# LeapLabTHU/LAUDNet

Measured on AMD Instinct MI355X. Metric: images/sec, LAUD-ResNet101 @224 bs256 (dynamic-inference hot path), higher is better.
Workload: dtype bf16x3 (fp32 tensors; each fp32 product = 3 bf16 MFMA products of hi/lo splits, fp32 accumulate)

## Files before the change

include/ldn_hip.h:

```cpp
#ifndef LDN_HIP_H
#define LDN_HIP_H

#include <stddef.h>
#include <stdint.h>

#ifdef __cplusplus
extern "C" {
#endif

#define LDN_OK 0
#define LDN_EINVAL (-1)
#define LDN_EHIP (-2)

const char* ldn_last_error(void);
int ldn_version(void);
int ldn_debug_violations(int* count, int* first_code, int reset);
int ldn_plan_timeouts(int* count, int reset);
const int* ldn_fault_flag(void);
int ldn_device_cus(int* cus);
#define LDN_MATH_DEFAULT (-1)
#define LDN_MATH_FP32 0
#define LDN_MATH_BF16X3 1
int ldn_default_math_mode(void);

// ... 77 lines not shown
                      double static_flops, int n_blocks, float* st_out, float* perc, float* flops, void* stream);

int ldn_conv_image(const float* a, int lda, int B, int Hi, int Wi, int ksize, int stride, int Ho, int Wo,
                   const float* w, int cin, int cout, const int32_t* k_idx, const int32_t* k_cnt, int kgran,
                   const int32_t* n_idx, const int32_t* n_cnt, const float* scale, const float* shift,
                   int shift_classes, const float* post_sub, int relu, const float* residual, int ldr,
                   float* out, int ldo, float* colsum, int out_format, int math_mode, void* stream);

int ldn_bottleneck_head(const float* x, int ldx, int B, int HW, int cin, const void* w1_split, int width,
                        const int32_t* ch_idx, const int32_t* ch_cnt, const float* scale1, const float* shift1,
                        const float* post_sub1, void* h1_split, int ldh, void* stream);
int ldn_bottleneck_head_f32(const float* x, int ldx, int B, int HW, int cin, const float* w1, int width,
                            const int32_t* ch_idx, const int32_t* ch_cnt, const float* scale1, const float* shift1,
                            const float* post_sub1, float* h1, int ldh, void* stream);
int ldn_bottleneck_tail_f32(const void* h1, int ldh, int B, int H, int Wd, int stride, int width, const void* w2_pairs_f32,
                            const void* w3_pairs_f32, int cout, const int32_t* ch_idx, const int32_t* ch_cnt, const float* scale2,
                            const float* shift2_tab, const float* post_sub2, const float* shift3, const float* residual,
                            int ldr, float* out, int ldo, float* colsum, void* stream);
int ldn_bottleneck_tail_splits(int H, int Wd, int width, int stride);
int ldn_bottleneck_tail(const void* h1_split, int ldh, int B, int H, int Wd, int stride, int width, const void* w2_pairs,
                        const void* w3_pairs, int cout, const int32_t* ch_idx, const int32_t* ch_cnt, const float* scale2,
                        const float* shift2_tab, const float* post_sub2, const float* shift3, const float* residual,
                        int ldr, float* out, int ldo, float* colsum, void* stream);
size_t ldn_x_split_bytes(size_t pixels, int cin);
int ldn_bottleneck_head_split(const float* x, int ldx, int B, int HW, int cin, const void* w1_split, int width,
                              const int32_t* ch_idx, const int32_t* ch_cnt, const float* scale1, const float* shift1,
                              const float* post_sub1, void* h1_split, int ldh, void* x_split, void* stream);
int ldn_bottleneck_tail_proj_fits(int H, int Wd, int width, int cin);
int ldn_bottleneck_tail_proj(const void* h1_split, int ldh, int B, int H, int Wd, int width, const void* w2_pairs,
                             const void* w3_pairs, int cout, const int32_t* ch_idx, const int32_t* ch_cnt, const float* scale2,
                             const float* shift2_tab, const float* post_sub2, const float* shift3d, const void* x_split,
                             int cin, const void* wd_pairs, float* out, int ldo, float* colsum, void* stream);

int ldn_bottleneck_smallmap_fits(int H, int Wd, int cin, int width, int cout);
int ldn_bottleneck_smallmap(const float* x, int ldx, int B, int H, int Wd, int cin, int width, const void* w1_split,
                            const void* w2_pairs, const void* w3_pairs, int cout, const int32_t* ch_idx, const int32_t* ch_cnt,
                            const float* scale1, const float* shift1, const float* post_sub1, const float* scale2,
                            const float* shift2_tab, const float* post_sub2, const float* shift3, const float* residual, int ldr,
                            float* out, int ldo, float* colsum, void* stream);

typedef struct ldn_chain_block {
    const void* w1_split; const float* scale1; const float* shift1; const float* post_sub1;
    const void* w2_pairs; const void* w3_pairs; const float* scale2; const float* shift2_tab; const float* post_sub2;
    const float* shift3;
    const float* mw1; const float* mb1; const float* mw2; const float* mb2;
} ldn_chain_block;
int ldn_bottleneck_chain_fits(int H, int Wd, int C, int width, int hidden, int G);
int ldn_bottleneck_chain(const float* x_in, float* x_work, int ldx, int B, int H, int Wd, int C, int width,
                         const ldn_chain_block* blocks, int nblocks, int hidden, int G, int gran, const float* gap_in,
                         int gap_splits, float* colsum, float* masks, int32_t* ch_idx, int32_t* ch_cnt, void* h1_split,
                         int ldh, void* stream);
int ldn_bottleneck_chain_f32(const float* x_in, float* x_work, int ldx, int B, int H, int Wd, int C, int width,
                         const ldn_chain_block* blocks, int nblocks, int hidden, int G, int gran, const float* gap_in,
                         int gap_splits, float* colsum, float* masks, int32_t* ch_idx, int32_t* ch_cnt, float* h1,
                         int ldh, void* stream);

size_t ldn_stem_weight_bytes(int cout);
int ldn_stem_conv_pool(const float* x, int B, int H, int W, const void* w_frag, const float* shift, int cout, float* out,
                       int Hp, int Wp, void* stream);
int ldn_stem_gap_splits(int H, int W);
int ldn_stem_conv_pool_gap(const float* x, int B, int H, int W, const void* w_frag, const float* shift, int cout,
                           float* out, int Hp, int Wp, float* gap, void* stream);

size_t ldn_stem3_weight_bytes(int cout);
int ldn_stem3_conv(const float* x, int B, int H, int W, const void* w_frag, const float* shift, int cout, int relu, float* out,
                   int Ho, int Wo, void* stream);
// ... 49 lines not shown
```

laudnet_amd/_lib.py:

```python
from __future__ import annotations

import ctypes as C
import os

import torch

_PKG = os.path.dirname(os.path.abspath(__file__))
LIB_PATH = os.environ.get("LDN_LIB_PATH", os.path.join(_PKG, "libldn_hip.so"))

_P = C.c_void_p
_I = C.c_int

SIGNATURES = {
    "ldn_last_error": ([], C.c_char_p),
    "ldn_version": ([], _I),
    "ldn_debug_violations": ([C.POINTER(_I), C.POINTER(_I), _I], _I),
    "ldn_plan_timeouts": ([C.POINTER(_I), _I], _I),
    "ldn_fault_flag": ([], C.POINTER(_I)),
    "ldn_device_cus": ([C.POINTER(_I)], _I),
    "ldn_default_math_mode": ([], _I),
    "ldn_spatial_masker": ([_P, _I, _I, _I, _I, _P, _P, _I, _I, _P, _P, _P, _P, _P, _P], _I),
    "ldn_spatial_masker_workspace_bytes": ([_I, _I, _I, _I, _I], C.c_size_t),
    "ldn_mask_to_index": ([_P, _I, _I, _I, _I, _I, _I, _P, _P, _P, _P, _P, _P, _P, _P, _P, _P, _P], _I),
    "ldn_mask_to_index_workspace_bytes": ([_I, _I, _I, _I], C.c_size_t),
# ... 27 lines not shown
    "ldn_grouped16_weight_bytes": ([_I], C.c_size_t),
    "ldn_grouped16_conv3x3_rows": ([_P, _I, _P, _P, _I, _P, _I, _P, _P, _I, _P, _I, _P], _I),
    "ldn_grouped16_images_fit": ([_I, _I, _I], _I),
    "ldn_grouped16_conv3x3_images": ([_P, _I, _P, _I, _I, _I, _I, _I, _I, _P, _I, _P, _P, _I, _P, _I, _P], _I),
    "ldn_plan_work_zeroed": ([_I], _I),
    "ldn_coarsen_cell_means": ([_P, _I, _I, _I, _P, _P], _I),
    "ldn_grouped16_images_bands": ([_I, _I, _I, _I, _I], _I),
    "ldn_grouped16_conv3x3_images_gap": ([_P, _I, _P, _I, _I, _I, _I, _I, _I, _P, _I, _P, _P, _I, _P, _I, _P, _P], _I),
    "ldn_se_gate_slots": ([_P, _I, _P, _I, _I, _I, _I, _P, _P, _P, _P, _P, _P], _I),
    "ldn_conv_rows_gated": ([_P, _I, _P, _I, _P, _I, _I, _P, _P, _I, _P, _P, _P, _I, _P, _I, _P, _I, _P], _I),
    "ldn_grouped_conv3x3_image": ([_P, _I, _I, _I, _I, _I, _I, _I, _P, _I, _I, _P, _P, _P, _P, _I, _P, _I, _P], _I),
    "ldn_se_packed": ([_P, _I, _P, _I, _I, _I, _P, _P, _P, _P, _P, _P, _I, _P, _P], _I),
    "ldn_se_packed_workspace_bytes": ([_I, _I, _I], C.c_size_t),
    "ldn_conv_image": ([_P, _I, _I, _I, _I, _I, _I, _I, _I, _P, _I, _I, _P, _P, _I, _P, _P, _P, _P, _I, _P, _I,
                        _P, _I, _P, _I, _P, _I, _I, _P], _I),
    "ldn_bottleneck_head": ([_P, _I, _I, _I, _I, _P, _I, _P, _P, _P, _P, _P, _P, _I, _P], _I),
    "ldn_bottleneck_head_f32": ([_P, _I, _I, _I, _I, _P, _I, _P, _P, _P, _P, _P, _P, _I, _P], _I),
    "ldn_bottleneck_tail_splits": ([_I, _I, _I, _I], _I),
    "ldn_bottleneck_tail": ([_P, _I, _I, _I, _I, _I, _I, _P, _P, _I, _P, _P, _P, _P, _P, _P, _P, _I, _P, _I, _P, _P], _I),
    "ldn_bottleneck_tail_f32": ([_P, _I, _I, _I, _I, _I, _I, _P, _P, _I, _P, _P, _P, _P, _P, _P, _P, _I, _P, _I, _P, _P], _I),
    "ldn_x_split_bytes": ([C.c_size_t, _I], C.c_size_t),
    "ldn_bottleneck_head_split": ([_P, _I, _I, _I, _I, _P, _I, _P, _P, _P, _P, _P, _P, _I, _P, _P], _I),
    "ldn_bottleneck_tail_proj_fits": ([_I, _I, _I, _I], _I),
    "ldn_bottleneck_tail_proj": ([_P, _I, _I, _I, _I, _I, _P, _P, _I, _P, _P, _P, _P, _P, _P, _P, _I, _P, _P, _I, _P, _P], _I),
    "ldn_stem_weight_bytes": ([_I], C.c_size_t),
    "ldn_stem_conv_pool": ([_P, _I, _I, _I, _P, _P, _I, _P, _I, _I, _P], _I),
    "ldn_stem_gap_splits": ([_I, _I], _I),
    "ldn_stem_conv_pool_gap": ([_P, _I, _I, _I, _P, _P, _I, _P, _I, _I, _P, _P], _I),
    "ldn_stem3_weight_bytes": ([_I], C.c_size_t),
    "ldn_stem3_conv": ([_P, _I, _I, _I, _P, _P, _I, _I, _P, _I, _I, _P], _I),
    "ldn_packed_mha": ([_P, _I, _P, _P, _I, _I, _I, _I, C.c_float, _P, _I, _P], _I),
    "ldn_packed_mha_heads": ([_P, _I, _P, _P, _I, _I, _I, _I, C.c_float, _P, _P, _I, _P], _I),
    "ldn_bottleneck_chain_fits": ([_I, _I, _I, _I, _I, _I], _I),
    "ldn_bottleneck_smallmap_fits": ([_I, _I, _I, _I, _I], _I),
    "ldn_bottleneck_smallmap": ([_P, _I, _I, _I, _I, _I, _I, _P, _P, _P, _I, _P, _P, _P, _P, _P, _P, _P, _P, _P, _P, _I, _P, _I, _P, _P], _I),
    "ldn_bottleneck_chain": ([_P, _P, _I, _I, _I, _I, _I, _I, _P, _I, _I, _I, _I, _P, _I, _P, _P, _P, _P, _P, _I, _P], _I),
    "ldn_bottleneck_chain_f32": ([_P, _P, _I, _I, _I, _I, _I, _I, _P, _I, _I, _I, _I, _P, _I, _P, _P, _P, _P, _P, _I, _P], _I),
}

_lib = None


class LdnError(RuntimeError):
    pass


def load():
    global _lib
    if _lib is not None:
        return _lib
    if not os.path.exists(LIB_PATH):
        raise LdnError(f"{LIB_PATH} not found: build it with `python -m laudnet_amd.build` "
                       "(laudnet_amd has no CPU or PyTorch fallback for the hot path)")
    lib = C.CDLL(LIB_PATH)
    for name, (argtypes, restype) in SIGNATURES.items():
        fn = getattr(lib, name)
        fn.argtypes = argtypes
        fn.restype = restype
    _lib = lib
    return lib


def ptr(t):
    if t is None:
        return None
    return C.c_void_p(t.data_ptr())
# ... 55 lines not shown
```

laudnet_amd/csrc/ldn_small.hip:

```cpp
#include <type_traits>

#include "ldn_common.h"

namespace ldn {

typedef __bf16 bf16x8 __attribute__((ext_vector_type(8)));
typedef __bf16 bf16x2 __attribute__((ext_vector_type(2)));
typedef unsigned u32x2 __attribute__((ext_vector_type(2)));
typedef unsigned u32x4 __attribute__((ext_vector_type(4)));

struct SmallArgs {
    const float* x; int ldx;
    int B, H, Wd, HW, cin, W, cout;
    const unsigned char* w1s;
    const unsigned char* w2p;
    const unsigned char* w3p;
    const int32_t* k_idx; const int32_t* k_cnt;
    const float* sc1; const float* sh1; const float* ps1;
    const float* sc2; const float* sh2; const float* ps2;
    const float* sh3;
    const float* residual; int ldr; float* out; int ldo;
    float* colsum;
};

__device__ __attribute__((aligned(16))) float g_small_zero[4] = {0.f, 0.f, 0.f, 0.f};

#ifndef SM_ABLATE
#define SM_ABLATE 0
#endif
#ifdef LDN_TRACE
__device__ unsigned long long* g_small_trace = nullptr;
#define ST(x) x = __builtin_amdgcn_s_memtime();
// ... 93 lines not shown
    const int slot32 = 16 * g.w2row;
    if (SM_FORCE_K16 == 0 && 3 * slot32 <= g.space) { g.nks2 = 2; g.slot2 = slot32; g.d2 = g.space / slot32 < 3 ? g.space / slot32 : 3; }
    else { g.nks2 = 1; g.slot2 = 8 * g.w2row; g.d2 = g.space / g.slot2 < 4 ? g.space / g.slot2 : 4; }
    g.d3 = g.space / 32768 < 3 ? g.space / 32768 : 3;
    return g;
}

__device__ __forceinline__ void store_presplit(unsigned char* act, int HW, int j, int pm, int h, int qd, const f32x4 v) {
    const bf16x2 h0 = {(__bf16)v[0], (__bf16)v[1]}, h1 = {(__bf16)v[2], (__bf16)v[3]};
    const bf16x2 l0 = {(__bf16)(v[0] - (float)h0[0]), (__bf16)(v[1] - (float)h0[1])};
    const bf16x2 l1 = {(__bf16)(v[2] - (float)h1[0]), (__bf16)(v[3] - (float)h1[1])};
    const u32x2 hi = {__builtin_bit_cast(unsigned, h0), __builtin_bit_cast(unsigned, h1)};
    const u32x2 lo = {__builtin_bit_cast(unsigned, l0), __builtin_bit_cast(unsigned, l1)};
    const unsigned sw = ((unsigned)pm >> 1) & 7u;
    unsigned char* row = act + (size_t)j * HW * 128 + pm * 128;
    *reinterpret_cast<u32x2*>(row + (((2u * qd) ^ sw) << 4) + 8 * h) = hi;
    *reinterpret_cast<u32x2*>(row + (((2u * qd + 1u) ^ sw) << 4) + 8 * h) = lo;
}

__device__ __forceinline__ float half_sum_dpp(float v) {
    auto dpp = [](float x, auto ctrl, auto rmask) {
        return __builtin_bit_cast(float, __builtin_amdgcn_update_dpp(0, __builtin_bit_cast(int, x), decltype(ctrl)::value, decltype(rmask)::value, 0xf, false));
    };
    v += dpp(v, std::integral_constant<int, 0xB1>{}, std::integral_constant<int, 0xf>{});
    v += dpp(v, std::integral_constant<int, 0x4E>{}, std::integral_constant<int, 0xf>{});
    v += dpp(v, std::integral_constant<int, 0x141>{}, std::integral_constant<int, 0xf>{});
    v += dpp(v, std::integral_constant<int, 0x140>{}, std::integral_constant<int, 0xf>{});
    v += dpp(v, std::integral_constant<int, 0x142>{}, std::integral_constant<int, 0xa>{});
    return v;
}

}

__global__ __launch_bounds__(512, 2) void k_smallmap(const SmallArgs p) {
    extern __shared__ __attribute__((aligned(16))) unsigned char smem[];
    const int tid = threadIdx.x, lane = tid & 63;
    const int wave = __builtin_amdgcn_readfirstlane(tid >> 6);
    const int l31 = lane & 31, h = lane >> 5;
    const int t = wave & 1, q = wave >> 1;
    const int b = blockIdx.x;
    const int W = p.W, HW = p.HW;
#ifdef LDN_TRACE
    unsigned long long ts[6] = {0, 0, 0, 0, 0, 0}, ta = 0, tb = 0, wt[3] = {0, 0, 0}, ct[3] = {0, 0, 0}, x3[3] = {0, 0, 0};
    ST(ts[0])
#endif
    int* const s_kidx = reinterpret_cast<int*>(smem);
    unsigned char* const s_act = smem + S_ACT_OFF;

    const int Kb = min(p.k_cnt[b], W);
    const int nsub = __builtin_amdgcn_readfirstlane(ceil_div(Kb, 32));
    const int Kp = nsub * 32;
    for (int i = tid; i < W + 32; i += 512) s_kidx[i] = i < Kb ? p.k_idx[(size_t)b * W + i] : -1;
    if (tid < 32) reinterpret_cast<float*>(smem + S_ZERO_OFF)[tid] = 0.f;
    LDN_DCHECK(p.k_cnt[b] >= 0 && p.k_cnt[b] <= W && (p.k_cnt[b] & 1) == 0, 701);
    if (tid < Kb) {
        const int ch = p.k_idx[(size_t)b * W + tid];
        LDN_DCHECK(ch >= 0 && ch < W, 702);
        LDN_DCHECK((tid & 1) ? (ch == p.k_idx[(size_t)b * W + tid - 1] + 1) : ((ch & 1) == 0), 703);
        LDN_DCHECK(tid == 0 || ch > p.k_idx[(size_t)b * W + tid - 1], 704);
    }
    __syncthreads();

    SmallGeom G = small_geom(HW, nsub);
    G.d2 = __builtin_amdgcn_readfirstlane(G.d2); G.d3 = __builtin_amdgcn_readfirstlane(G.d3);
    G.nks2 = __builtin_amdgcn_readfirstlane(G.nks2); G.slot2 = __builtin_amdgcn_readfirstlane(G.slot2);
    G.w2row = __builtin_amdgcn_readfirstlane(G.w2row); G.ring_off = __builtin_amdgcn_readfirstlane(G.ring_off);
    const int pm = 32 * t + l31;
// ... 152 lines not shown
                    }
                }
            }
#pragma unroll
            for (int i = 0; i < 4; ++i)
#pragma unroll
                for (int r = 0; r < 16; ++r) acc[i][r] = 0.f;
            lds_barrier();
            ST(ts[2])
        }

        {
            const int oy = pm / p.Wd, ox = pm - oy * p.Wd;
            unsigned tmask = 0;
#pragma unroll
            for (int tp = 0; tp < 9; ++tp) {
                const int iy = oy + tp / 3 - 1, ix = ox + tp % 3 - 1;
                const bool ok = pvalid && iy >= 0 && iy < p.H && ix >= 0 && ix < p.Wd;
                tmask |= ok ? (1u << tp) : 0u;
            }
            const int cls = (((oy - 1 < 0) | ((oy + 1 >= p.H) << 1)) * 4 + ((ox - 1 < 0) | ((ox + 1 >= p.Wd) << 1)));
            const int nks = G.nks2, D = G.d2, W2ROW = G.w2row, slotB = G.slot2;
            const int nf = W2ROW / 1024;
            const int per = nks == 2 ? 1 : 2;
            const int nchunks = nsub * 9 * per;
            const int ipc = nks * nf;
            int npo[4];
#pragma unroll
            for (int f = 0; f < 4; ++f) {
                const int v = 64 * f + lane;
                const int ch = 2 * v < Kb ? s_kidx[2 * v] : -1;
                npo[f] = ch >= 0 ? (ch >> 1) * 16 : -1;
            }
            if (D > 1) {
                unsigned vo[4];
#pragma unroll
                for (int f = 0; f < 4; ++f) {
                    const int v = 64 * f + lane;
                    vo[f] = (unsigned)((s_kidx[2 * v < Kb ? 2 * v : 0] >> 1) * 16 + (3 - f) * 1024);
                }
                const long tapstride = (long)(W / 2) * (W / 2) * 16;
                const unsigned ring_bytes = (unsigned)(D * slotB);
                int is = 0, itp = 0, ihf = 0; unsigned foff = 0;
                int rbv[2];
                auto load_rb = [&]() {
#pragma unroll
                    for (int e = 0; e < 2; ++e)
                        rbv[e] = (s_kidx[min(32 * min(is, nsub - 1) + (nks == 2 ? 4 * wave + 2 * e : 16 * e + 2 * wave), Kb - 2)] >> 1) * (W / 2) * 16;
                };
                load_rb();
                auto row_dma = [&](const void* sbase, unsigned lds) {
                    if (nf == 3) dma16_gather_row<3>(vo, sbase, lds);
                    else if (nf == 4) dma16_gather_row<4>(vo, sbase, lds);
                    else if (nf == 2) dma16_gather_row<2>(vo, sbase, lds);
                    else dma16_gather_row<1>(vo, sbase, lds);
                };
                auto issue = [&]() {
                    const unsigned char* tapbase = p.w2p + (long)itp * tapstride - 3072;
                    const unsigned slot = lds_ring + foff;
                    if (nks == 2) {
                        row_dma(uniform_ptr(tapbase + __builtin_amdgcn_readfirstlane(rbv[0])), slot + (2 * wave) * W2ROW);
                        row_dma(uniform_ptr(tapbase + __builtin_amdgcn_readfirstlane(rbv[1])), slot + (2 * wave + 1) * W2ROW);
                    } else {
                        row_dma(uniform_ptr(tapbase + __builtin_amdgcn_readfirstlane(ihf ? rbv[1] : rbv[0])), slot + wave * W2ROW);
                    }
                    foff += slotB; if (foff == ring_bytes) foff = 0;
                    if (++ihf == per) { ihf = 0; if (++itp == 9) { itp = 0; ++is; load_rb(); } }
// ... 179 lines not shown
#pragma unroll
                                for (int qq = 0; qq < 4; ++qq) e[i][qq] = *reinterpret_cast<const u32x2*>(ws + a_lane + qq * W2ROW + jo[i]);
#pragma unroll
                            for (int i = 0; i < 4; ++i) {
                                if (q + 4 * i < nsub) {
                                    const u32x4 ahu = {e[i][0][0], e[i][1][0], e[i][2][0], e[i][3][0]};
                                    const u32x4 alu = {e[i][0][1], e[i][1][1], e[i][2][1], e[i][3][1]};
                                    const bf16x8 ah = __builtin_bit_cast(bf16x8, ahu), al = __builtin_bit_cast(bf16x8, alu);
                                    acc[i] = __builtin_amdgcn_mfma_f32_32x32x16_bf16(al, bh, acc[i], 0, 0, 0);
                                    acc[i] = __builtin_amdgcn_mfma_f32_32x32x16_bf16(ah, bl, acc[i], 0, 0, 0);
                                    acc[i] = __builtin_amdgcn_mfma_f32_32x32x16_bf16(ah, bh, acc[i], 0, 0, 0);
                                }
                                if (D > 1) issue_part(i);
                            }
                            if (D > 1) issue_advance();
                        }
                        ST(tb)
                        ST_ADD(ct[1], ta, tb)
                    }
                }
            }
            }
            wait_vm_n<0>();
            lds_barrier();
            ST(ts[3])
            float* const s_tab = reinterpret_cast<float*>(smem + G.ring_off);
            for (int i = tid; i < 18 * Kp; i += 512) {
                const int k = i / Kp, n = i - k * Kp;
                const int ch = s_kidx[n];
                const float* src = k == 0 ? p.sc2 : (k == 1 ? p.ps2 : p.sh2 + (size_t)(k - 2) * W);
                s_tab[i] = ch >= 0 ? src[ch] : 0.f;
            }
            lds_barrier();
            if (pvalid) {
#pragma unroll
                for (int i = 0; i < 4; ++i) {
                    const int j = q + 4 * i;
                    if (j < nsub) {
#pragma unroll
                        for (int qd = 0; qd < 4; ++qd) {
                            const int n0 = 32 * j + 8 * qd + 4 * h;
                            const f32x4 sc = *reinterpret_cast<const f32x4*>(s_tab + n0);
                            const f32x4 ps = *reinterpret_cast<const f32x4*>(s_tab + Kp + n0);
                            const f32x4 sh = *reinterpret_cast<const f32x4*>(s_tab + (2 + cls) * Kp + n0);
                            f32x4 v;
#pragma unroll
                            for (int e = 0; e < 4; ++e) v[e] = fmaxf(acc[i][4 * qd + e] * sc[e] + sh[e], 0.f) - ps[e];
                            store_presplit(s_act, HW, j, pm, h, qd, v);
                        }
                    }
                }
            }
            lds_barrier();
            ST(ts[4])
        }
    }

    {
        const int D = G.d3;
        const int nk16 = Kp / 16;
        const int ngroups = ceil_div(p.cout, 512);
        const int nchunks = ngroups * nk16;
        int ig = 0, iks = 0, ioff = 0, coff = 0;
        const unsigned char* i3base = nullptr;
        auto issue_begin = [&]() {
            i3base = nullptr;
            if (ig < ngroups && nk16 > 0) {
                const int kch = s_kidx[16 * iks + 2 * wave];
                if (kch >= 0) i3base = p.w3p + ((long)(kch >> 1) * p.cout + 512 * ig + 2 * lane) * 8;
            }
        };
        auto issue_part = [&](int f) {
            const unsigned slot = lds_ring + ioff;
            const unsigned char* src = (i3base && 512 * ig + 128 * f < p.cout) ? i3base + f * 1024 : reinterpret_cast<const unsigned char*>(g_small_zero);
            dma16(src, slot + wave * 4096 + f * 1024);
        };
        auto issue_advance = [&]() {
            ioff += 32768; if (ioff == D * 32768) ioff = 0;
            if (ig < ngroups && nk16 > 0) { if (++iks == nk16) { iks = 0; ++ig; } }
        };
        auto issue = [&]() {
            issue_begin();
#pragma unroll
            for (int f = 0; f < 4; ++f) issue_part(f);
            issue_advance();
        };
        const bool fast3 = D > 1 && (p.cout & 511) == 0 && nk16 > 0;
        if (D > 1 && !fast3) for (int c = 0; c < D - 1; ++c) issue();
        const unsigned rx = ((unsigned)prow >> 1) & 7u;
        const unsigned a_lane = (unsigned)(4 * h * 4096 + l31 * 8);
        auto group_epilogue = [&](int g) {
// ... 151 lines not shown
                        const u32x4 ahu = {e[i][0][0], e[i][1][0], e[i][2][0], e[i][3][0]};
                        const u32x4 alu = {e[i][0][1], e[i][1][1], e[i][2][1], e[i][3][1]};
                        const bf16x8 ah = __builtin_bit_cast(bf16x8, ahu), al = __builtin_bit_cast(bf16x8, alu);
                        acc[i] = __builtin_amdgcn_mfma_f32_32x32x16_bf16(al, bh, acc[i], 0, 0, 0);
                        acc[i] = __builtin_amdgcn_mfma_f32_32x32x16_bf16(ah, bl, acc[i], 0, 0, 0);
                        acc[i] = __builtin_amdgcn_mfma_f32_32x32x16_bf16(ah, bh, acc[i], 0, 0, 0);
                    }
                    if (D > 1) issue_part(i);
                }
                if (D > 1) issue_advance();
            }
            if (active) group_epilogue(g);
        }
        }
        wait_vm_n<0>();
#ifdef LDN_TRACE
        ST(ts[5])
        if (g_small_trace && lane == 0) {
            unsigned long long* r = g_small_trace + ((size_t)b * 8 + wave) * 16;
            for (int i = 0; i < 6; ++i) r[i] = ts[i];
            for (int i = 0; i < 3; ++i) { r[6 + i] = wt[i]; r[9 + i] = ct[i]; }
            r[12] = nsub; r[13] = x3[0]; r[14] = x3[1]; r[15] = x3[2];
        }
#endif
        if (p.colsum && !active) {
            for (int cch = 128 * q + lane * 2; cch < p.cout; cch += 512) {
                p.colsum[((size_t)b * 2 + t) * p.cout + cch] = 0.f;
                p.colsum[((size_t)b * 2 + t) * p.cout + cch + 1] = 0.f;
            }
        }
    }
}

LDN_DEFINE_TU_VIOLATIONS(tu_violations_small)

static bool small_fits(int HW, int cin, int width, int cout) {
    if (HW < 1 || HW > 64 || width < 64 || width > 512 || width % 64 || cin < 32 || cin % 32 || cout < 128 || cout % 128) return false;
    const int nsub = width / 32;
    const SmallGeom g = small_geom(HW, nsub);
    if (S_ACT_OFF + g.act_bytes > S_LDS - S_TAB1_BYTES) return false;
    if (g.space < 18 * width * 4) return false;
    if (g.d2 < 1 || g.d3 < 1) return false;
    if (2 * (64 + width) * 128 > S_LDS - S_ACT_OFF) return false;
    return true;
}

}

using namespace ldn;

#ifdef LDN_TRACE
extern "C" int ldn_debug_set_small_trace(void* buf) {
    unsigned long long* q = static_cast<unsigned long long*>(buf);
    return hipMemcpyToSymbol(HIP_SYMBOL(g_small_trace), &q, sizeof(q)) == hipSuccess ? 0 : -2;
}
#endif

extern "C" int ldn_bottleneck_smallmap_fits(int H, int Wd, int cin, int width, int cout) {
    if (H < 1 || Wd < 1) return 0;
    return small_fits(H * Wd, cin, width, cout) ? 1 : 0;
}

extern "C" int ldn_bottleneck_smallmap(const float* x, int ldx, int B, int H, int Wd, int cin, int width, const void* w1_split,
                                       const void* w2_pairs, const void* w3_pairs, int cout, const int32_t* ch_idx,
                                       const int32_t* ch_cnt, const float* scale1, const float* shift1, const float* post_sub1,
                                       const float* scale2, const float* shift2_tab, const float* post_sub2, const float* shift3,
                                       const float* residual, int ldr, float* out, int ldo, float* colsum, void* stream) {
    LDN_REQUIRE(x && w1_split && w2_pairs && w3_pairs && ch_idx && ch_cnt && scale1 && shift1 && post_sub1 && scale2 && shift2_tab &&
                post_sub2 && shift3 && out, "ldn_bottleneck_smallmap: null pointer");
    LDN_REQUIRE(B > 0 && H > 0 && Wd > 0, "ldn_bottleneck_smallmap: bad geometry");
    LDN_REQUIRE(small_fits(H * Wd, cin, width, cout),
                "ldn_bottleneck_smallmap: a %dx%d map with cin %d, width %d, cout %d does not fit the workgroup (ldn_bottleneck_smallmap_fits == 0)",
                H, Wd, cin, width, cout);
    LDN_REQUIRE(ldx >= cin && ldx % 4 == 0 && ldo >= cout && ldo % 4 == 0 && (!residual || (ldr >= cout && ldr % 4 == 0)),
                "ldn_bottleneck_smallmap: bad ldx / ldo / ldr");
    LDN_REQUIRE((uintptr_t)x % 16 == 0 && (uintptr_t)w1_split % 16 == 0 && (uintptr_t)w2_pairs % 16 == 0 && (uintptr_t)w3_pairs % 16 == 0 &&
                (uintptr_t)out % 16 == 0 && (uintptr_t)residual % 16 == 0 && (uintptr_t)shift3 % 16 == 0 && (uintptr_t)colsum % 16 == 0,
                "ldn_bottleneck_smallmap: pointers must be 16-byte aligned");
    SmallArgs a{};
    a.x = x; a.ldx = ldx; a.B = B; a.H = H; a.Wd = Wd; a.HW = H * Wd; a.cin = cin; a.W = width; a.cout = cout;
    a.w1s = static_cast<const unsigned char*>(w1_split);
    a.w2p = static_cast<const unsigned char*>(w2_pairs);
    a.w3p = static_cast<const unsigned char*>(w3_pairs);
    a.k_idx = ch_idx; a.k_cnt = ch_cnt;
    a.sc1 = scale1; a.sh1 = shift1; a.ps1 = post_sub1; a.sc2 = scale2; a.sh2 = shift2_tab; a.ps2 = post_sub2; a.sh3 = shift3;
    a.residual = residual; a.ldr = ldr; a.out = out; a.ldo = ldo; a.colsum = colsum;
    LDN_REQUIRE(allow_dynamic_lds(reinterpret_cast<const void*>(&k_smallmap), S_LDS), "k_smallmap: cannot reserve %d B of LDS", S_LDS);
    hipLaunchKernelGGL(k_smallmap, dim3((unsigned)B), dim3(512), S_LDS, static_cast<hipStream_t>(stream), a);
    LDN_CHECK_LAUNCH("k_smallmap");
    return LDN_OK;
}
```

laudnet_amd/ops.py:

```python
from __future__ import annotations

import os
import threading
import weakref
from dataclasses import dataclass

import torch

from . import _lib as L


def _f32c(t, what):
    if t is None:
        return None
    if t.dtype != torch.float32 or not t.is_contiguous():
        raise L.LdnError(f"{what}: expected a contiguous float32 tensor, got {t.dtype} strides {t.stride()}")
    return t


def _f32rows(t, what):
    if t is None:
        return None
    if t.dtype != torch.float32 or t.dim() != 2 or t.stride(1) != 1 or t.data_ptr() % 16 != 0:
        raise L.LdnError(f"{what}: expected a 16-byte aligned float32 matrix with contiguous rows, got {t.dtype} strides {t.stride()}")
# ... 871 lines not shown
    v = (t[:, :, :, 0] + t[:, :, :, 1]).permute(0, 3, 1, 2, 4).reshape(-1, cin)
    return v[:pixels]


def bottleneck_tail_proj_fits(H, W, width, cin):
    return bool(L.load().ldn_bottleneck_tail_proj_fits(H, W, width, cin))


def bottleneck_tail_proj(h1_split, w2_pairs, w3_pairs, ch_idx, ch_cnt, scale2, shift2_tab, post_sub2, shift3d, x_split, wd_pairs,
                         out_nhwc, *, colsum=None):
    L.require_device(h1_split, w2_pairs, w3_pairs, x_split, wd_pairs, out_nhwc)
    lib = L.load()
    B, H, Wd, ldh = h1_split.shape
    width = ch_idx.shape[1]
    cout = out_nhwc.shape[-1]
    cin = wd_pairs.shape[0] * 2
    if tuple(out_nhwc.shape) != (B, H, Wd, cout) or x_split.numel() * 4 < lib.ldn_x_split_bytes(B * H * Wd, cin) or not x_split.is_contiguous():
        raise L.LdnError(f"bottleneck_tail_proj: out must be [B={B}, {H}, {Wd}, cout], x_split the buffer bottleneck_head filled")
    for t in (w2_pairs, w3_pairs, wd_pairs):
        if t.dtype != torch.bfloat16 or not t.is_contiguous():
            raise L.LdnError("bottleneck_tail_proj: w2_pairs / w3_pairs / wd_pairs must be the contiguous bf16 tensors of pack_w2_pairs / pack_w3_pairs")
    L.check(lib.ldn_bottleneck_tail_proj(L.ptr(_f32c(h1_split, "h1")), ldh, B, H, Wd, width, L.ptr(w2_pairs), L.ptr(w3_pairs), cout,
                                         L.ptr(_i32c(ch_idx, "ch_idx")), L.ptr(_i32c(ch_cnt, "ch_cnt")), L.ptr(_f32c(scale2, "scale2")),
                                         L.ptr(_f32c(shift2_tab, "shift2_tab")), L.ptr(_f32c(post_sub2, "post_sub2")),
                                         L.ptr(_f32c(shift3d, "shift3d")), L.ptr(x_split), cin, L.ptr(wd_pairs),
                                         L.ptr(_f32c(out_nhwc, "out")), cout, L.ptr(colsum), L.stream_ptr(out_nhwc)), "ldn_bottleneck_tail_proj")
    return out_nhwc


def bottleneck_smallmap_fits(H, W, cin, width, cout):
    return bool(L.load().ldn_bottleneck_smallmap_fits(H, W, cin, width, cout))


def bottleneck_smallmap(x_nhwc, w1_split, w2_pairs, w3_pairs, ch_idx, ch_cnt, scale1, shift1, post_sub1, scale2, shift2_tab, post_sub2,
                        shift3, out_nhwc, *, residual=None, colsum=None):
    L.require_device(x_nhwc, w1_split, w2_pairs, w3_pairs, out_nhwc)
    lib = L.load()
    B, H, Wd, cin = x_nhwc.shape
    width = ch_idx.shape[1]
    cout = out_nhwc.shape[-1]
    if tuple(out_nhwc.shape) != (B, H, Wd, cout) or (residual is not None and tuple(residual.shape) != (B, H, Wd, cout)):
        raise L.LdnError(f"bottleneck_smallmap: out / residual must be [B={B}, {H}, {Wd}, cout]")
    if colsum is not None and (tuple(colsum.shape) != (B, 2, cout) or not colsum.is_contiguous()):
        raise L.LdnError("bottleneck_smallmap: colsum must be a contiguous [B, 2, cout] tensor")
    for w in (w1_split, w2_pairs, w3_pairs):
        if w.dtype != torch.bfloat16 or not w.is_contiguous():
            raise L.LdnError("bottleneck_smallmap: weights must be the contiguous bf16 tensors of pack_w1_split / pack_w2_pairs / pack_w3_pairs")
    L.check(lib.ldn_bottleneck_smallmap(L.ptr(_f32c(x_nhwc, "x")), cin, B, H, Wd, cin, width, L.ptr(w1_split), L.ptr(w2_pairs),
                                        L.ptr(w3_pairs), cout, L.ptr(_i32c(ch_idx, "ch_idx")), L.ptr(_i32c(ch_cnt, "ch_cnt")),
                                        L.ptr(_f32c(scale1, "scale1")), L.ptr(_f32c(shift1, "shift1")), L.ptr(_f32c(post_sub1, "post_sub1")),
                                        L.ptr(_f32c(scale2, "scale2")), L.ptr(_f32c(shift2_tab, "shift2_tab")),
                                        L.ptr(_f32c(post_sub2, "post_sub2")), L.ptr(_f32c(shift3, "shift3")), L.ptr(residual),
                                        cout if residual is not None else 0, L.ptr(_f32c(out_nhwc, "out")), cout, L.ptr(colsum),
                                        L.stream_ptr(out_nhwc)), "ldn_bottleneck_smallmap")
    return out_nhwc


def pack_stem_weights(w_scaled):
    cout = w_scaled.shape[0]
    if tuple(w_scaled.shape[1:]) != (3, 7, 7) or cout % 32:
        raise L.LdnError("pack_stem_weights: expected [cout % 32 == 0, 3, 7, 7]")
    w = w_scaled.detach().float().permute(0, 2, 3, 1).reshape(cout, 7, 21)
    k = torch.zeros(cout, 8, 24, device=w.device, dtype=torch.float32)
    k[:, :7, :21] = w
    k = k.reshape(cout, 24, 8)[:, :22]
    k = k.reshape(cout // 32, 32, 11, 2, 8)
# ... 79 lines not shown
```

Before: 23590.

## Add register-pipelined weight streaming variant of smallmap bottleneck kernel

Adds a templated variant of the small-feature-map bottleneck kernel. In it, the 3x3 conv and the final 1x1 conv stream weight fragments directly from global memory into a 4-deep register ring. These loads are software-pipelined against double-buffered LDS activation fragments feeding bf16x3 MFMAs, with each wave owning 64-pixel by 32/64-channel tiles. The goal is to hide global weight-load latency and avoid the previous staging path. It is selected by default through an environment variable. The trade-off is higher register pressure at 512 threads with 2 blocks per CU, which could cause spills.

```diff
diff --git a/include/ldn_hip.h b/include/ldn_hip.h
--- a/include/ldn_hip.h
+++ b/include/ldn_hip.h
@@ -133,6 +133,7 @@
                              const float* shift2_tab, const float* post_sub2, const float* shift3d, const void* x_split,
                              int cin, const void* wd_pairs, float* out, int ldo, float* colsum, void* stream);
 
+int ldn_bottleneck_smallmap_form(void);
 int ldn_bottleneck_smallmap_fits(int H, int Wd, int cin, int width, int cout);
 int ldn_bottleneck_smallmap(const float* x, int ldx, int B, int H, int Wd, int cin, int width, const void* w1_split,
                             const void* w2_pairs, const void* w3_pairs, int cout, const int32_t* ch_idx, const int32_t* ch_cnt,
diff --git a/laudnet_amd/_lib.py b/laudnet_amd/_lib.py
--- a/laudnet_amd/_lib.py
+++ b/laudnet_amd/_lib.py
@@ -83,6 +83,7 @@
     "ldn_packed_mha": ([_P, _I, _P, _P, _I, _I, _I, _I, C.c_float, _P, _I, _P], _I),
     "ldn_packed_mha_heads": ([_P, _I, _P, _P, _I, _I, _I, _I, C.c_float, _P, _P, _I, _P], _I),
     "ldn_bottleneck_chain_fits": ([_I, _I, _I, _I, _I, _I], _I),
+    "ldn_bottleneck_smallmap_form": ([], _I),
     "ldn_bottleneck_smallmap_fits": ([_I, _I, _I, _I, _I], _I),
     "ldn_bottleneck_smallmap": ([_P, _I, _I, _I, _I, _I, _I, _P, _P, _P, _I, _P, _P, _P, _P, _P, _P, _P, _P, _P, _P, _I, _P, _I, _P, _P], _I),
     "ldn_bottleneck_chain": ([_P, _P, _I, _I, _I, _I, _I, _I, _P, _I, _I, _I, _I, _P, _I, _P, _P, _P, _P, _P, _I, _P], _I),
diff --git a/laudnet_amd/csrc/ldn_small.hip b/laudnet_amd/csrc/ldn_small.hip
--- a/laudnet_amd/csrc/ldn_small.hip
+++ b/laudnet_amd/csrc/ldn_small.hip
@@ -1,3 +1,4 @@
+#include <stdlib.h>
 #include <type_traits>
 
 #include "ldn_common.h"
@@ -157,7 +158,7 @@
 
 }
 
-__global__ __launch_bounds__(512, 2) void k_smallmap(const SmallArgs p) {
+template <int REGW> __device__ __forceinline__ void small_body(const SmallArgs p) {
     extern __shared__ __attribute__((aligned(16))) unsigned char smem[];
     const int tid = threadIdx.x, lane = tid & 63;
     const int wave = __builtin_amdgcn_readfirstlane(tid >> 6);
@@ -376,7 +377,120 @@
                 const int ch = 2 * v < Kb ? s_kidx[2 * v] : -1;
                 npo[f] = ch >= 0 ? (ch >> 1) * 16 : -1;
             }
-            if (D > 1) {
+            if constexpr ((REGW & 2) != 0) {
+                constexpr int RD = 4;
+                const int nv2 = nsub > wave ? (nsub - wave + 7) / 8 : 0;
+                const unsigned tapstride = (unsigned)((W / 2) * (W / 2) * 16);
+                const unsigned rowbytes = (unsigned)((W / 2) * 16);
+                unsigned tm2[2]; int pm2[2];
+#pragma unroll
+                for (int tt = 0; tt < 2; ++tt) {
+                    pm2[tt] = 32 * tt + l31;
+                    const int oy2 = pm2[tt] / p.Wd, ox2 = pm2[tt] - oy2 * p.Wd;
+                    tm2[tt] = 0;
+#pragma unroll
+                    for (int tp = 0; tp < 9; ++tp) {
+                        const int iy = oy2 + tp / 3 - 1, ix = ox2 + tp % 3 - 1;
+                        const bool ok = pm2[tt] < HW && iy >= 0 && iy < p.H && ix >= 0 && ix < p.Wd;
+                        tm2[tt] |= ok ? (1u << tp) : 0u;
+                    }
+                }
+                auto run = [&](auto NVc) {
+                    constexpr int NV = decltype(NVc)::value;
+                    if constexpr (NV > 0) {
+                        struct BF { bf16x8 bh[2], bl[2]; };
+                        u32x2 qa[RD][NV][4];
+                        unsigned noff[NV];
+#pragma unroll
+                        for (int u = 0; u < NV; ++u) {
+                            const int n = 32 * (wave + 8 * u) + l31, ne = n & ~1;
+                            noff[u] = (unsigned)((s_kidx[ne < Kb ? ne : 0] >> 1) * 16 + (n & 1) * 8);
+                        }
+                        int ls = 0, ltp = 0, lkk = 0;
+                        unsigned ltap = 0, lro[2][4];
+                        auto load_ro = [&]() {
+#pragma unroll
+                            for (int kk = 0; kk < 2; ++kk)
+#pragma unroll
+                                for (int qq = 0; qq < 4; ++qq)
+                                    lro[kk][qq] = (unsigned)(s_kidx[min(32 * ls + 16 * kk + 8 * h + 2 * qq, Kb - 2)] >> 1) * rowbytes;
+                        };
+                        load_ro();
+                        auto issue = [&](u32x2 (&qx)[NV][4]) {
+                            if (ls < nsub) {
+#pragma unroll
+                                for (int qq = 0; qq < 4; ++qq) {
+                                    const unsigned char* src = p.w2p + (ltap + (lkk ? lro[1][qq] : lro[0][qq]));
+#pragma unroll
+                                    for (int u = 0; u < NV; ++u) qx[u][qq] = *reinterpret_cast<const u32x2*>(src + noff[u]);
+                                }
+                                if (++lkk == 2) {
+                                    lkk = 0; ltap += tapstride;
+                                    if (++ltp == 9) { ltp = 0; ltap = 0; ++ls; if (ls < nsub) load_ro(); }
+                                }
+                            }
+                        };
+                        auto load_b = [&](BF& f, int s2, int tp, int kk) {
+                            const int ty = (tp * 11) >> 5;
+                            const unsigned sl = 2u * (2u * kk + h);
+#pragma unroll
+                            for (int tt = 0; tt < 2; ++tt) {
+                                const int r = ((tm2[tt] >> tp) & 1u) ? pm2[tt] + (ty - 1) * p.Wd + (tp - 3 * ty - 1) : -1;
+                                const unsigned char* hrow = r >= 0 ? s_act + (size_t)s2 * HW * 128 + r * 128 : smem + S_ZERO_OFF;
+                                const unsigned rx = r >= 0 ? ((unsigned)r >> 1) & 7u : 0u;
+                                f.bh[tt] = *reinterpret_cast<const bf16x8*>(hrow + ((sl ^ rx) << 4));
+                                f.bl[tt] = *reinterpret_cast<const bf16x8*>(hrow + (((sl + 1) ^ rx) << 4));
+                            }
+                        };
+                        int cs = 0, ctp = 0, ckk = 0;
+                        auto step = [&](u32x2 (&qx)[NV][4], const BF& bc, BF& bn) {
+                            if (++ckk == 2) { ckk = 0; if (++ctp == 9) { ctp = 0; if (cs + 1 < nsub) ++cs; } }
+                            load_b(bn, cs, ctp, ckk);
+                            bf16x8 ah[NV], al[NV];
+#pragma unroll
+                            for (int u = 0; u < NV; ++u) {
+                                const u32x4 ahu = {qx[u][0][0], qx[u][1][0], qx[u][2][0], qx[u][3][0]};
+                                const u32x4 alu = {qx[u][0][1], qx[u][1][1], qx[u][2][1], qx[u][3][1]};
+                                ah[u] = __builtin_bit_cast(bf16x8, ahu); al[u] = __builtin_bit_cast(bf16x8, alu);
+                            }
+                            issue(qx);
+#pragma unroll
+                            for (int tt = 0; tt < 2; ++tt)
+#pragma unroll
+                                for (int u = 0; u < NV; ++u)
+                                    acc[2 * tt + u] = __builtin_amdgcn_mfma_f32_32x32x16_bf16(al[u], bc.bh[tt], acc[2 * tt + u], 0, 0, 0);
+#pragma unroll
+                            for (int tt = 0; tt < 2; ++tt)
+#pragma unroll
+                                for (int u = 0; u < NV; ++u)
+                                    acc[2 * tt + u] = __builtin_amdgcn_mfma_f32_32x32x16_bf16(ah[u], bc.bl[tt], acc[2 * tt + u], 0, 0, 0);
+#pragma unroll
+                            for (int tt = 0; tt < 2; ++tt)
+#pragma unroll
+                                for (int u = 0; u < NV; ++u)
+                                    acc[2 * tt + u] = __builtin_amdgcn_mfma_f32_32x32x16_bf16(ah[u], bc.bh[tt], acc[2 * tt + u], 0, 0, 0);
+                        };
+                        const int T = nsub * 18;
+#pragma unroll
+                        for (int d = 0; d < RD; ++d) issue(qa[d]);
+                        BF b0, b1;
+                        load_b(b0, 0, 0, 0);
+#pragma unroll 1
+                        for (int base = 0; base < T; base += RD) {
+#pragma unroll
+                            for (int d = 0; d < RD; ++d)
+                                if (base + d < T) {
+                                    if (d & 1) step(qa[d], b1, b0); else step(qa[d], b0, b1);
+                                }
+                        }
+                    }
+                };
+                switch (nv2) {
+                    case 0: break;
+                    case 1: run(std::integral_constant<int, 1>{}); break;
+                    default: run(std::integral_constant<int, 2>{}); break;
+                }
+            } else if (D > 1) {
                 unsigned vo[4];
 #pragma unroll
                 for (int f = 0; f < 4; ++f) {
@@ -622,7 +736,33 @@
                 s_tab[i] = ch >= 0 ? src[ch] : 0.f;
             }
             lds_barrier();
-            if (pvalid) {
+            if constexpr ((REGW & 2) != 0) {
+#pragma unroll
+                for (int tt = 0; tt < 2; ++tt) {
+                    const int pmx = 32 * tt + l31;
+                    if (pmx < HW) {
+                        const int oy2 = pmx / p.Wd, ox2 = pmx - oy2 * p.Wd;
+                        const int cls2 = (((oy2 - 1 < 0) | ((oy2 + 1 >= p.H) << 1)) * 4 + ((ox2 - 1 < 0) | ((ox2 + 1 >= p.Wd) << 1)));
+#pragma unroll
+                        for (int u = 0; u < 2; ++u) {
+                            const int j = wave + 8 * u;
+                            if (j < nsub) {
+#pragma unroll
+                                for (int qd = 0; qd < 4; ++qd) {
+                                    const int n0 = 32 * j + 8 * qd + 4 * h;
+                                    const f32x4 sc = *reinterpret_cast<const f32x4*>(s_tab + n0);
+                                    const f32x4 ps = *reinterpret_cast<const f32x4*>(s_tab + Kp + n0);
+                                    const f32x4 sh = *reinterpret_cast<const f32x4*>(s_tab + (2 + cls2) * Kp + n0);
+                                    f32x4 v;
+#pragma unroll
+                                    for (int e = 0; e < 4; ++e) v[e] = fmaxf(acc[2 * tt + u][4 * qd + e] * sc[e] + sh[e], 0.f) - ps[e];
+                                    store_presplit(s_act, HW, j, pmx, h, qd, v);
+                                }
+                            }
+                        }
+                    }
+                }
+            } else if (pvalid) {
 #pragma unroll
                 for (int i = 0; i < 4; ++i) {
                     const int j = q + 4 * i;
@@ -646,7 +786,118 @@
         }
     }
 
-    {
+    if constexpr ((REGW & 1) != 0) {
+        constexpr int RD = 4;
+        const int nk16 = Kp / 16;
+        const int npairs = p.cout / 64;
+        const int npass = __builtin_amdgcn_readfirstlane(npairs > wave ? (npairs - wave + 7) / 8 : 0);
+        bool pv2[2]; int pm2[2]; unsigned bo2[2];
+#pragma unroll
+        for (int tt = 0; tt < 2; ++tt) {
+            pm2[tt] = 32 * tt + l31;
+            pv2[tt] = pm2[tt] < HW;
+            const unsigned pr = pv2[tt] ? (unsigned)pm2[tt] : 0u;
+            bo2[tt] = pr * 128u + (((2u * h) ^ ((pr >> 1) & 7u)) << 4);
+        }
+        auto pass_epilogue = [&](int i) {
+#pragma unroll
+            for (int tt = 0; tt < 2; ++tt)
+#pragma unroll
+                for (int u = 0; u < 2; ++u) {
+                    const int c0 = 64 * (wave + 8 * i) + 32 * u;
+                    const int pmx = pm2[tt];
+                    const bool pvx = pv2[tt];
+                    f32x4 res[4], sh[4];
+#pragma unroll
+                    for (int qd = 0; qd < 4; ++qd) {
+                        const int cch = c0 + 8 * qd + 4 * h;
+                        const float* rsrc = (p.residual && pvx) ? p.residual + (img_row0 + pmx) * p.ldr + cch : g_small_zero;
+                        res[qd] = *reinterpret_cast<const f32x4*>(rsrc);
+                        sh[qd] = *reinterpret_cast<const f32x4*>(p.sh3 + cch);
+                    }
+#pragma unroll
+                    for (int qd = 0; qd < 4; ++qd) {
+                        const int cch = c0 + 8 * qd + 4 * h;
+                        f32x4 x;
+#pragma unroll
+                        for (int e = 0; e < 4; ++e) x[e] = fmaxf(acc[2 * tt + u][4 * qd + e] + sh[qd][e] + res[qd][e], 0.f);
+                        if (pvx) *reinterpret_cast<f32x4*>(p.out + (img_row0 + pmx) * p.ldo + cch) = x;
+                        if (p.colsum) {
+#pragma unroll
+                            for (int e = 0; e < 4; ++e) x[e] = half_sum_dpp(pvx ? x[e] : 0.f);
+                            if (l31 == 31) *reinterpret_cast<f32x4*>(p.colsum + ((size_t)b * 2 + tt) * p.cout + cch) = x;
+                        }
+                    }
+#pragma unroll
+                    for (int r = 0; r < 16; ++r) acc[2 * tt + u][r] = 0.f;
+                }
+        };
+#pragma unroll
+        for (int i = 0; i < 4; ++i)
+#pragma unroll
+            for (int r = 0; r < 16; ++r) acc[i][r] = 0.f;
+        if (nk16 == 0) {
+            for (int i = 0; i < npass; ++i) pass_epilogue(i);
+        } else {
+            struct BF { bf16x8 bh[2], bl[2]; };
+            u32x2 qa[RD][2][4];
+            int li = 0, lks = 0;
+            auto issue = [&](u32x2 (&qx)[2][4]) {
+                if (li < npass) {
+                    const unsigned c8 = (unsigned)(64 * (wave + 8 * li) + l31) * 8u;
+#pragma unroll
+                    for (int qq = 0; qq < 4; ++qq) {
+                        const int kch = s_kidx[min(16 * lks + 8 * h + 2 * qq, Kb - 2)];
+                        const unsigned char* src = p.w3p + ((unsigned)(kch >> 1) * (unsigned)p.cout * 8u + c8);
+                        qx[0][qq] = *reinterpret_cast<const u32x2*>(src);
+                        qx[1][qq] = *reinterpret_cast<const u32x2*>(src + 256);
+                    }
+                    if (++lks == nk16) { lks = 0; ++li; }
+                }
+            };
+            auto load_b = [&](BF& f, int ks) {
+                const unsigned char* hs = s_act + (size_t)(ks >> 1) * HW * 128;
+#pragma unroll
+                for (int tt = 0; tt < 2; ++tt) {
+                    const unsigned bofs = bo2[tt] ^ ((unsigned)(ks & 1) << 6);
+                    f.bh[tt] = *reinterpret_cast<const bf16x8*>(hs + bofs);
+                    f.bl[tt] = *reinterpret_cast<const bf16x8*>(hs + (bofs ^ 16u));
+                }
+            };
+            int ci = 0, cks = 0;
+            auto step = [&](u32x2 (&qx)[2][4], const BF& bc, BF& bn) {
+                load_b(bn, cks + 1 == nk16 ? 0 : cks + 1);
+                bf16x8 ah[2], al[2];
+#pragma unroll
+                for (int u = 0; u < 2; ++u) {
+                    const u32x4 ahu = {qx[u][0][0], qx[u][1][0], qx[u][2][0], qx[u][3][0]};
+                    const u32x4 alu = {qx[u][0][1], qx[u][1][1], qx[u][2][1], qx[u][3][1]};
+                    ah[u] = __builtin_bit_cast(bf16x8, ahu); al[u] = __builtin_bit_cast(bf16x8, alu);
+                }
+                issue(qx);
+#pragma unroll
+                for (int a = 0; a < 4; ++a) acc[a] = __builtin_amdgcn_mfma_f32_32x32x16_bf16(al[a & 1], bc.bh[a >> 1], acc[a], 0, 0, 0);
+#pragma unroll
+                for (int a = 0; a < 4; ++a) acc[a] = __builtin_amdgcn_mfma_f32_32x32x16_bf16(ah[a & 1], bc.bl[a >> 1], acc[a], 0, 0, 0);
+#pragma unroll
+                for (int a = 0; a < 4; ++a) acc[a] = __builtin_amdgcn_mfma_f32_32x32x16_bf16(ah[a & 1], bc.bh[a >> 1], acc[a], 0, 0, 0);
+                if (++cks == nk16) { cks = 0; pass_epilogue(ci); ++ci; }
+            };
+            const int T = npass * nk16;
+#pragma unroll
+            for (int d = 0; d < RD; ++d) issue(qa[d]);
+            BF b0, b1;
+            load_b(b0, 0);
+#pragma unroll 1
+            for (int base = 0; base < T; base += RD) {
+#pragma unroll
+                for (int d = 0; d < RD; ++d)
+                    if (base + d < T) {
+                        if (d & 1) step(qa[d], b1, b0); else step(qa[d], b0, b1);
+                    }
+            }
+        }
+    } else {
         const int D = G.d3;
         const int nk16 = Kp / 16;
         const int ngroups = ceil_div(p.cout, 512);
@@ -864,6 +1115,9 @@
     }
 }
 
+__global__ __launch_bounds__(512, 2) void k_smallmap(const SmallArgs p) { small_body<0>(p); }
+template <int REGW> __global__ __launch_bounds__(512, 2) void k_smallmap_regw(const SmallArgs p) { small_body<REGW>(p); }
+
 LDN_DEFINE_TU_VIOLATIONS(tu_violations_small)
 
 static bool small_fits(int HW, int cin, int width, int cout) {
@@ -887,6 +1141,19 @@
     return hipMemcpyToSymbol(HIP_SYMBOL(g_small_trace), &q, sizeof(q)) == hipSuccess ? 0 : -2;
 }
 #endif
+
+#ifndef LDN_SMALL_REGW_DEFAULT
+#define LDN_SMALL_REGW_DEFAULT 1
+#endif
+static int small_regw() {
+    static const int form = [] {
+        const char* e = getenv("LDN_SMALL_REGW");
+        return (e && *e ? atoi(e) : LDN_SMALL_REGW_DEFAULT) != 0 ? 1 : 0;
+    }();
+    return form;
+}
+
+extern "C" int ldn_bottleneck_smallmap_form(void) { return small_regw(); }
 
 extern "C" int ldn_bottleneck_smallmap_fits(int H, int Wd, int cin, int width, int cout) {
     if (H < 1 || Wd < 1) return 0;
@@ -917,8 +1184,11 @@
     a.k_idx = ch_idx; a.k_cnt = ch_cnt;
     a.sc1 = scale1; a.sh1 = shift1; a.ps1 = post_sub1; a.sc2 = scale2; a.sh2 = shift2_tab; a.ps2 = post_sub2; a.sh3 = shift3;
     a.residual = residual; a.ldr = ldr; a.out = out; a.ldo = ldo; a.colsum = colsum;
-    LDN_REQUIRE(allow_dynamic_lds(reinterpret_cast<const void*>(&k_smallmap), S_LDS), "k_smallmap: cannot reserve %d B of LDS", S_LDS);
-    hipLaunchKernelGGL(k_smallmap, dim3((unsigned)B), dim3(512), S_LDS, static_cast<hipStream_t>(stream), a);
-    LDN_CHECK_LAUNCH("k_smallmap");
-    return LDN_OK;
-}
+    auto launch = [&](auto kernel) {
+        LDN_REQUIRE(allow_dynamic_lds(reinterpret_cast<const void*>(kernel), S_LDS), "k_smallmap: cannot reserve %d B of LDS", S_LDS);
+        hipLaunchKernelGGL(kernel, dim3((unsigned)B), dim3(512), S_LDS, static_cast<hipStream_t>(stream), a);
+        LDN_CHECK_LAUNCH("k_smallmap");
+        return LDN_OK;
+    };
+    return small_regw() ? launch(&k_smallmap_regw<3>) : launch(&k_smallmap);
+}
diff --git a/laudnet_amd/ops.py b/laudnet_amd/ops.py
--- a/laudnet_amd/ops.py
+++ b/laudnet_amd/ops.py
@@ -927,6 +927,10 @@
     return bool(L.load().ldn_bottleneck_smallmap_fits(H, W, cin, width, cout))
 
 
+def bottleneck_smallmap_form():
+    return int(L.load().ldn_bottleneck_smallmap_form())
+
+
 def bottleneck_smallmap(x_nhwc, w1_split, w2_pairs, w3_pairs, ch_idx, ch_cnt, scale1, shift1, post_sub1, scale2, shift2_tab, post_sub2,
                         shift3, out_nhwc, *, residual=None, colsum=None):
     L.require_device(x_nhwc, w1_split, w2_pairs, w3_pairs, out_nhwc)
```

Result: no change. 23580, median of 2 (-0.0%).
